# adamjorr/kbbq-py

Measured on NVIDIA B200. Metric: bases/sec recalibrated (table build + apply), higher is better.
Workload: dtype u8 in/out, u32->int64 counts, f64 model

## Files before the change

### include/kbbq_b200.h

```cpp
#ifndef KBBQ_B200_H
#define KBBQ_B200_H

#include <stddef.h>
#include <stdint.h>

#ifdef __cplusplus
extern "C" {
#endif

#define KBBQ_NQ 43
#define KBBQ_NDINUC 16

#define KBBQ_OK 0
#define KBBQ_E_ARG (-1)
#define KBBQ_E_CUDA (-2)
#define KBBQ_E_WORKSPACE (-3)
#define KBBQ_E_DATA (-4)
#define KBBQ_E_IO (-5)
#define KBBQ_E_FORMAT (-6)
#define KBBQ_E_RAGGED (-7)
#define KBBQ_E_NAME_FIELD (-8)
#define KBBQ_E_NAME_RG (-9)
#define KBBQ_E_NAME_MISMATCH (-10)
#define KBBQ_E_PEER (-11)
// ... 3 lines not shown
#define KBBQ_FLAG_BAD_BASE 2
#define KBBQ_FLAG_RG_RANGE 4
#define KBBQ_FLAG_SEGMENTS 8
#define KBBQ_FLAG_KMER_FULL 16

int kbbq_abi_version(void);
const char *kbbq_strerror(int code);
const char *kbbq_last_cuda_error(void);

int64_t kbbq_pos_table_elems(int L, int R);
int64_t kbbq_din_table_elems(int R);

int kbbq_workspace_bytes(int64_t N, int L, int R, size_t *bytes);

int kbbq_build(const uint8_t *seq_dev, const uint8_t *qual_dev, const uint8_t *corr_dev,
               const uint16_t *rg_dev, const uint8_t *second_dev, int64_t N, int L, int R,
               int minscore, int64_t *pos_errs_dev, int64_t *pos_total_dev, int64_t *din_errs_dev,
               int64_t *din_total_dev, void *workspace_dev, size_t workspace_bytes,
               int *status_dev, int path, void *stream);

int kbbq_marginals(const int64_t *pos_errs_dev, const int64_t *pos_total_dev, int L, int R,
                   int64_t *q_errs_dev, int64_t *q_total_dev, int64_t *rg_errs_dev,
                   int64_t *rg_total_dev, int64_t *meanq_dev, void *stream);

int kbbq_delta_q(const int64_t *prior_q_dev, const int64_t *numerrs_dev,
                 const int64_t *numtotal_dev, int64_t n, int64_t *delta_dev, void *stream);

int kbbq_posterior_q_real(const double *prior_q_dev, const int64_t *numerrs_dev,
                          const int64_t *numtotal_dev, int64_t n, int64_t *posterior_dev, void *stream);

int kbbq_bam_workspace_bytes(int64_t N, int L, int R, size_t *bytes);
int kbbq_build_bam(const uint8_t *seq_dev, const uint8_t *qual_dev, const uint8_t *err_dev,
                   const uint8_t *skip_dev, const uint16_t *rg_dev, const uint8_t *flags_dev,
                   const uint16_t *aln_start_dev, const uint16_t *aln_end_dev, int64_t N, int L, int R,
                   int minscore, int64_t *pos_errs_dev, int64_t *pos_total_dev, int64_t *din_errs_dev,
                   int64_t *din_total_dev, void *workspace_dev, size_t workspace_bytes, int *status_dev,
                   void *stream);
int kbbq_apply_bam(const uint8_t *seq_dev, const uint8_t *qual_dev, const uint16_t *rg_dev,
                   const uint8_t *flags_dev, int64_t N, int L, int R, int minscore,
                   const int64_t *meanq_dev, const int64_t *rgdq_dev, const int64_t *qdq_dev,
                   const int64_t *posdq_dev, const int64_t *dindq_dev, int nq, int ndin1,
                   uint8_t *out_qual_dev, void *workspace_dev, size_t workspace_bytes, int *status_dev,
                   void *stream);

int kbbq_calibration_counts(const uint8_t *qual_dev, const uint8_t *err_dev, const uint8_t *seq_dev,
                            const uint8_t *corr_dev, const uint8_t *skip_dev, int64_t n,
// ... 190 lines not shown
```

### kbbq-py_b200/csrc/host_api.cu

```cuda
#include <algorithm>
#include <atomic>
#include <chrono>
#include <condition_variable>
#include <memory>
#include <mutex>
#include <sched.h>
#include <stdlib.h>
#include <string.h>
#include <sys/mman.h>
#include <sys/stat.h>
#include <fcntl.h>
#include <thread>
#include <unistd.h>
#include <vector>

#include "common.cuh"

using namespace kbbq;

namespace {

#define KBBQ_TRY(x) do { int rc_ = (x); if (rc_) return rc_; } while (0)

constexpr int MAX_DEVICES = 16;
// ... 453 lines not shown
    if (st & KBBQ_FLAG_KMER_FULL) return KBBQ_E_DATA;
    S->kmer_t = min_count > 0 ? min_count : kbbq_kmer_min_count(hist);
    S->kmer_stage = KMER_READY;
    if (hist_out) memcpy(hist_out, hist, sizeof(hist));
    if (t_used) *t_used = S->kmer_t;
    return KBBQ_OK;
}

int build_chunk_kmer_async(kbbq_session *S, const uint8_t *seq, const uint8_t *qual, const uint16_t *rg,
                           const uint8_t *second, int64_t n) {
    if (S->kmer_stage != KMER_READY || n < 0 || n > S->C) return KBBQ_E_ARG;
    if (n == 0) return KBBQ_OK;
    if (!seq || !qual) return KBBQ_E_ARG;
    const int64_t k = S->built++;
    KBBQ_TRY(build_chunk_upload(S, k, seq, qual, rg, second, n, false, true));
    return build_chunk_finish(S, k, seq, nullptr, rg != nullptr, second != nullptr, n, false);
}

int model_async(kbbq_session *S) {
    const int L = S->L, R = S->R;
    const size_t npos = (size_t)R * NQ * 2 * L, ndin = (size_t)R * NQ * 16;
    int64_t *pe = S->summed ? S->d_sum : S->d_tab, *pt = pe + npos, *de = pt + npos, *dt = de + ndin;
    const ModelPtrs &mp = S->mp;
    KBBQ_TRY(kbbq_marginals(pe, pt, L, R, mp.q_errs, mp.q_total, mp.rg_errs, mp.rg_total, mp.meanq, S->s_comp));
    KBBQ_TRY(kbbq_get_delta_qs(mp.meanq, mp.rg_errs, mp.rg_total, mp.q_errs, mp.q_total, pe, pt, de, dt, R, NQ, 2 * L, 16,
                               mp.rgdq, mp.qdq, mp.posdq, mp.dindq, S->s_comp));
    return KBBQ_OK;
}

int apply_and_download(kbbq_session *S, const uint8_t *d_seq, const uint8_t *d_qual, const uint16_t *d_rg,
                       const uint8_t *d_sec, const uint32_t *seg, const uint32_t *dest, int64_t n, uint8_t *out_host) {
    const int L = S->L, R = S->R;
    OutSlot &o = S->down[S->applied++ & 1];
    const ModelPtrs &mp = S->mp;
    KBBQ_CUDA(cudaStreamWaitEvent(S->s_comp, o.drained, 0));
    if (S->segmode) {
        KBBQ_TRY(kbbq_apply_segmented(d_seq, d_qual, seg, S->rowsC, L, R, S->minscore, mp.meanq, mp.rgdq, mp.qdq, mp.posdq,
                                      mp.dindq, NQ, 17, o.out_seg, S->d_ws, S->ws_bytes, S->d_status, S->s_comp));
        KBBQ_TRY(kbbq_unsegment_rows(o.out_seg, dest, n, L, S->rowsC, o.out, S->s_comp));
    } else {
        KBBQ_TRY(kbbq_apply(d_seq, d_qual, d_rg, d_sec, n, L, R, S->minscore, mp.meanq, mp.rgdq, mp.qdq, mp.posdq, mp.dindq,
                            NQ, 17, o.out, S->d_ws, S->ws_bytes, S->d_status, 0, S->s_comp));
    }
    KBBQ_CUDA(cudaEventRecord(o.applied, S->s_comp));
    KBBQ_CUDA(cudaStreamWaitEvent(S->s_down, o.applied, 0));
    KBBQ_CUDA(cudaMemcpyAsync(out_host, o.out, (size_t)n * L, cudaMemcpyDeviceToHost, S->s_down));
    S->d2h_bytes += n * L;
    KBBQ_CUDA(cudaEventRecord(o.drained, S->s_down));
    return KBBQ_OK;
// ... 1058 lines not shown
    const auto d_hist = c.scratch(256 * sizeof(uint64_t));
    const auto d_tab = c.scratch(ntab * 8);
    const auto d_model = c.scratch(nmodel * 8);
    const auto ws = c.scratch(ws_bytes);
    const auto table = c.scratch(table_bytes);
    bool ok = false;
    KBBQ_TRY(c.fits(&ok));
    if (!ok) return KBBQ_E_UNSUPPORTED;
    KBBQ_TRY(c.begin());
    uint64_t hist[256];
    int t = 0, st = 0;
    const int rc = kmer_errors_dev(d_seq, N, L, k, min_count, table, cap, (uint64_t *)(void *)d_hist,
                                   (uint32_t *)(void *)d_bits, c.status, hist, &t, &st);
    if (rc == KBBQ_E_DATA && status_out) *status_out = st;
    KBBQ_TRY(rc);
    if (min_count_used) *min_count_used = t;
    int64_t *pe = (int64_t *)(void *)d_tab, *pt = pe + npos, *de = pt + npos, *dt = de + ndin;
    const ModelPtrs mp = carve_model((int64_t *)(void *)d_model, L, R);
    uint8_t *corr = (uint8_t *)(void *)d_corr;
    KBBQ_CUDA(cudaMemset(pe, 0, ntab * 8));
    KBBQ_TRY(kbbq_expand_mismatch_bits(d_seq, (uint32_t *)(void *)d_bits, (int64_t)nb, corr, nullptr));
    KBBQ_TRY(kbbq_build(d_seq, d_qual, corr, d_rg, d_sec, N, L, R, minscore, pe, pt, de, dt, ws, ws_bytes, c.status, 0,
                        nullptr));
    KBBQ_TRY(kbbq_marginals(pe, pt, L, R, mp.q_errs, mp.q_total, mp.rg_errs, mp.rg_total, mp.meanq, nullptr));
    KBBQ_TRY(kbbq_get_delta_qs(mp.meanq, mp.rg_errs, mp.rg_total, mp.q_errs, mp.q_total, pe, pt, de, dt, R, NQ, 2 * L,
                               16, mp.rgdq, mp.qdq, mp.posdq, mp.dindq, nullptr));
    KBBQ_TRY(kbbq_apply(d_seq, d_qual, d_rg, d_sec, N, L, R, minscore, mp.meanq, mp.rgdq, mp.qdq, mp.posdq, mp.dindq, NQ,
                        17, d_out, ws, ws_bytes, c.status, KBBQ_APPLY_BASES_CHECKED, nullptr));
    if (tables_host) KBBQ_CUDA(cudaMemcpy(tables_host, pe, ntab * 8, cudaMemcpyDeviceToHost));
    if (deltas_host)
        KBBQ_CUDA(cudaMemcpy(deltas_host, mp.meanq, ((size_t)2 * R + (size_t)R * NQ * (1 + 2 * L + 17)) * 8,
                             cudaMemcpyDeviceToHost));
    return c.finish(status_out);
}

}
```

### kbbq-py_b200/csrc/kbbq_b200.cu

```cuda
#include <algorithm>
#include <mutex>
#include <stdlib.h>
#include <string.h>
#include <vector>

#include "apply.cuh"
#include "bam.cuh"
#include "build.cuh"
#include "calib.cuh"
#include "common.cuh"
#include "expand.cuh"
#include "kmer.cuh"
#include "model.cuh"
#include "prepare.cuh"
#include "segment.cuh"
#include "synth.cuh"

namespace kbbq {

std::atomic<long long> g_launches{0};
char g_last_cuda_error[256] = "";

static std::mutex g_const_mu;
static bool g_const_done[64];
// ... 128 lines not shown
        return KBBQ_OK;
    }
    const int64_t tail = (R == 1 && N > p->g.G) ? N % p->g.G : 0;
    if (tail) {
        p->N = N - tail;
        rc = generic(p->N, tail, 1);
        if (rc) return rc;
    }
    return run_prepare(rg, second, p->N, p->g.G, R, p->w, status, p->sms, p->sl.ngs, p->g.gbytes, p->sl.slot, st);
}

template <class Launch>
static int launch_bam_chunks(long long N, int L, const Launch &launch) {
    const unsigned int wmax = (unsigned int)((3 + L + 3) >> 2);
    const long long per = std::max<long long>(1, (long long)(0x7FFFFFFFu / wmax) / 256 * 256);
    for (long long r0 = 0; r0 < N; r0 += per) {
        const long long n = std::min<long long>(per, N - r0);
        launch((unsigned)((n * wmax + BAM_WARPS * 32 - 1) / (BAM_WARPS * 32)), r0, wmax);
        KBBQ_LAUNCHED();
    }
    return KBBQ_OK;
}

}

using namespace kbbq;

extern "C" {

int kbbq_abi_version(void) { return 1; }

const char *kbbq_strerror(int code) {
    switch (code) {
    case KBBQ_OK: return "ok";
    case KBBQ_E_ARG: return "bad argument";
    case KBBQ_E_CUDA: return "CUDA runtime error";
    case KBBQ_E_WORKSPACE: return "workspace too small";
    case KBBQ_E_DATA: return "input data error (see status flags)";
    case KBBQ_E_IO: return "FASTQ file could not be opened, read or written";
    case KBBQ_E_FORMAT: return "malformed FASTQ (4-line records expected)";
    case KBBQ_E_RAGGED: return "reads of unequal length";
    case KBBQ_E_NAME_FIELD: return "read name has no read-group field";
    case KBBQ_E_NAME_RG: return "read-group field does not start with RG";
    case KBBQ_E_NAME_MISMATCH: return "corrected read name does not start with the read name";
    case KBBQ_E_PEER: return "multi-GPU: peer access between the devices is not available";
    case KBBQ_E_UNSUPPORTED: return "not handled by this entry point (use the chunked driver)";
// ... 64 lines not shown
}

int kbbq_build(const uint8_t *seq, const uint8_t *qual, const uint8_t *corr, const uint16_t *rg,
               const uint8_t *second, int64_t N, int L, int R, int minscore, int64_t *pos_errs,
               int64_t *pos_total, int64_t *din_errs, int64_t *din_total, void *workspace,
               size_t workspace_bytes, int *status, int path, void *stream) {
    return build_impl(seq, qual, corr, rg, second, N, L, R, minscore, pos_errs, pos_total, din_errs, din_total,
                      workspace, workspace_bytes, status, path, stream, nullptr);
}

int kbbq_build_segmented(const uint8_t *seq, const uint8_t *qual, const uint8_t *corr, const uint32_t *seg,
                         int64_t rows_bound, int L, int R, int minscore, int64_t *pos_errs, int64_t *pos_total,
                         int64_t *din_errs, int64_t *din_total, void *workspace, size_t workspace_bytes, int *status,
                         void *stream) {
    if (!seg || rows_bound % SEG_ALIGN) return KBBQ_E_ARG;
    return build_impl(seq, qual, corr, nullptr, nullptr, rows_bound, L, R, minscore, pos_errs, pos_total, din_errs,
                      din_total, workspace, workspace_bytes, status, 1, stream, seg);
}

int kbbq_marginals(const int64_t *pos_errs, const int64_t *pos_total, int L, int R, int64_t *q_errs,
                   int64_t *q_total, int64_t *rg_errs, int64_t *rg_total, int64_t *meanq, void *stream) {
    if (L < 1 || R < 1 || !pos_errs || !pos_total || !q_errs || !q_total || !rg_errs || !rg_total || !meanq)
        return KBBQ_E_ARG;
    cudaStream_t st = (cudaStream_t)stream;
    int rc = upload_constants();
    if (rc) return rc;
    marginals_q_kernel<<<dim3(NQ, R), 128, 0, st>>>((const long long *)pos_errs, (const long long *)pos_total,
                                                   2 * L, (long long *)q_errs, (long long *)q_total);
    KBBQ_LAUNCHED();
    marginals_rg_kernel<<<R, 64, 0, st>>>((const long long *)q_errs, (const long long *)q_total, R,
                                                      (long long *)rg_errs, (long long *)rg_total, (long long *)meanq);
    KBBQ_LAUNCHED();
    return KBBQ_OK;
}

int kbbq_delta_q(const int64_t *prior_q, const int64_t *numerrs, const int64_t *numtotal, int64_t n,
                 int64_t *delta, void *stream) {
    if (n < 0 || (n > 0 && (!prior_q || !numerrs || !numtotal || !delta))) return KBBQ_E_ARG;
    if (n == 0) return KBBQ_OK;
    int rc = upload_constants();
    if (rc) return rc;
    delta_q_kernel<<<(unsigned)((n + 127) / 128), 128, 0, (cudaStream_t)stream>>>(
        (const long long *)prior_q, (const long long *)numerrs, (const long long *)numtotal, n, (long long *)delta);
    KBBQ_LAUNCHED();
    return KBBQ_OK;
}

int kbbq_posterior_q_real(const double *prior_q, const int64_t *numerrs, const int64_t *numtotal, int64_t n,
                          int64_t *posterior, void *stream) {
    if (n < 0 || (n > 0 && (!prior_q || !numerrs || !numtotal || !posterior))) return KBBQ_E_ARG;
    if (n == 0) return KBBQ_OK;
    int rc = upload_constants();
    if (rc) return rc;
    posterior_q_real_kernel<<<(unsigned)((n + 127) / 128), 128, 0, (cudaStream_t)stream>>>(
        prior_q, (const long long *)numerrs, (const long long *)numtotal, n, (long long *)posterior);
    KBBQ_LAUNCHED();
// ... 126 lines not shown
    const long long chunk = (long long)grid * CAL_THREADS * CAL_MAX_ITERS * 32;
    auto kern = err ? (skip ? calibration_kernel<true, true> : calibration_kernel<true, false>)
                    : (skip ? calibration_kernel<false, true> : calibration_kernel<false, false>);
    KBBQ_CUDA(cudaFuncSetAttribute(kern, cudaFuncAttributeMaxDynamicSharedMemorySize, CAL_SMEM));
    for (long long o = 0; o < n; o += chunk) {
        CalibArgs c = a;
        c.qual += o; if (err) c.err += o; else { c.seq += o; c.corr += o; } if (skip) c.skip += o;
        c.n = std::min<long long>(chunk, n - o);
        kern<<<grid, CAL_THREADS, CAL_SMEM, st>>>(c);
        KBBQ_LAUNCHED();
    }
    return KBBQ_OK;
}

int kbbq_get_delta_qs(const int64_t *meanq, const int64_t *rg_errs, const int64_t *rg_total,
                      const int64_t *q_errs, const int64_t *q_total, const int64_t *pos_errs,
                      const int64_t *pos_total, const int64_t *din_errs, const int64_t *din_total, int R,
                      int nq, int ncyc, int ndin, int64_t *rgdq, int64_t *qdq, int64_t *posdq,
                      int64_t *dindq, void *stream) {
    if (R < 1 || nq < 1 || ncyc < 0 || ndin < 0) return KBBQ_E_ARG;
    if (!meanq || !rg_errs || !rg_total || !q_errs || !q_total || !rgdq || !qdq) return KBBQ_E_ARG;
    if ((ncyc && (!pos_errs || !pos_total || !posdq)) || !dindq || (ndin && (!din_errs || !din_total)))
        return KBBQ_E_ARG;
    int rc = upload_constants();
    if (rc) return rc;
    cudaStream_t st = (cudaStream_t)stream;
    DeltaArgs a = {(const long long *)meanq, (const long long *)rg_errs, (const long long *)rg_total,
                   (const long long *)q_errs, (const long long *)q_total, (const long long *)pos_errs,
                   (const long long *)pos_total, (const long long *)din_errs, (const long long *)din_total,
                   R, nq, ncyc, ndin, (long long *)rgdq, (long long *)qdq, (long long *)posdq, (long long *)dindq};
    delta_levels12_kernel<<<R, 64, 0, st>>>(a);
    KBBQ_LAUNCHED();
    const long long cells = (long long)R * nq * (ncyc + ndin + 1);
    delta_level3_kernel<<<(unsigned)((cells + 127) / 128), 128, 0, st>>>(a);
    KBBQ_LAUNCHED();
    return KBBQ_OK;
}

static int apply_impl(const uint8_t *seq, const uint8_t *qual, const uint16_t *rg, const uint8_t *second, int64_t N,
                      int L, int R, int minscore, const int64_t *meanq, const int64_t *rgdq, const int64_t *qdq,
                      const int64_t *posdq, const int64_t *dindq, int nq, int ndin1, uint8_t *out_qual,
                      void *workspace, size_t workspace_bytes, int *status, int path, void *stream,
                      const unsigned int *seg_rows) {
    const bool segmode = seg_rows != nullptr;
    const bool validate = !(path & KBBQ_APPLY_BASES_CHECKED);
    path &= ~KBBQ_APPLY_BASES_CHECKED;
    if (N < 0 || L < 1 || R < 1 || R > 65535 || minscore < 0 || minscore >= NQ) return KBBQ_E_ARG;
    if (nq < 1 || nq > NQ || ndin1 < 16 || ndin1 > 64) return KBBQ_E_ARG;
    if (!meanq || !rgdq || !qdq || !posdq || !dindq || !status) return KBBQ_E_ARG;
    if (N == 0) return KBBQ_OK;
    if (!seq || !qual || !out_qual) return KBBQ_E_ARG;
    cudaStream_t st = (cudaStream_t)stream;
    Workspace w = carve_workspace(workspace, N, L, R);
    if (!workspace || workspace_bytes < w.bytes) return KBBQ_E_WORKSPACE;

    const long long fold_cells = (long long)R * NQ * (2 * L + 16);
    fold_kernel<<<(unsigned)((fold_cells + 255) / 256), 256, 0, st>>>(
        (const long long *)meanq, (const long long *)rgdq, (const long long *)qdq, (const long long *)posdq,
        (const long long *)dindq, R, nq, 2 * L, ndin1, w.fold_cyc, w.fold_din);
// ... 321 lines not shown
```

### kbbq-py_b200/csrc/model.cuh

```cuda
#pragma once
#include "common.cuh"

namespace kbbq {

__constant__ double c_lnp[NQ];
__constant__ double c_ln1mp[NQ];
__constant__ double c_prior[NQ];
__constant__ double c_p[NQ];
__constant__ double c_bound_hi[NQ];
__constant__ double c_bound_lo[NQ];

struct dd { double hi, lo; };
__device__ __forceinline__ dd two_sum(double a, double b) {
    double s = __dadd_rn(a, b), bb = __dsub_rn(s, a);
    double e = __dadd_rn(__dsub_rn(a, __dsub_rn(s, bb)), __dsub_rn(b, bb));
    return {s, e};
}
__device__ __forceinline__ dd two_prod(double a, double b) {
    double p = __dmul_rn(a, b);
    return {p, __fma_rn(a, b, -p)};
}
__device__ __forceinline__ dd dd_add(dd a, dd b) {
    dd s = two_sum(a.hi, b.hi);
    double lo = __dadd_rn(s.lo, __dadd_rn(a.lo, b.lo));
    return two_sum(s.hi, lo);
}
__device__ __forceinline__ dd dd_div_d(dd a, double b) {
    double q1 = __ddiv_rn(a.hi, b);
    dd p = two_prod(q1, b);
    double r = __dadd_rn(__dsub_rn(__dsub_rn(a.hi, p.hi), p.lo), a.lo);
    double q2 = __ddiv_rn(r, b);
    return two_sum(q1, q2);
}
__device__ __forceinline__ bool dd_le(dd a, double bh, double bl) {
    return a.hi < bh || (a.hi == bh && a.lo <= bl);
}

__global__ void marginals_q_kernel(const long long *pos_errs, const long long *pos_total, int L2,
                                   long long *q_errs, long long *q_total) {
    const int q = blockIdx.x, rg = blockIdx.y;
    const size_t base = ((size_t)rg * NQ + q) * L2;
    long long e = 0, t = 0;
    for (int c = threadIdx.x; c < L2; c += blockDim.x) { e += pos_errs[base + c]; t += pos_total[base + c]; }
    __shared__ long long se[32], st[32];
    for (int o = 16; o; o >>= 1) { e += __shfl_down_sync(0xFFFFFFFFu, e, o); t += __shfl_down_sync(0xFFFFFFFFu, t, o); }
    if ((threadIdx.x & 31) == 0) { se[threadIdx.x >> 5] = e; st[threadIdx.x >> 5] = t; }
    __syncthreads();
    if (threadIdx.x == 0) {
        e = 0; t = 0;
        for (int w = 0; w < (blockDim.x + 31) / 32; ++w) { e += se[w]; t += st[w]; }
        q_errs[rg * NQ + q] = e;
        q_total[rg * NQ + q] = t;
    }
}

__global__ void marginals_rg_kernel(const long long *q_errs, const long long *q_total, int R,
                                    long long *rg_errs, long long *rg_total, long long *meanq) {
    const int rg = blockIdx.x;
    __shared__ long long s_e[NQ], s_t[NQ];
    if (threadIdx.x < NQ) {
        s_e[threadIdx.x] = q_errs[rg * NQ + threadIdx.x];
        s_t[threadIdx.x] = q_total[rg * NQ + threadIdx.x];
    }
    __syncthreads();
    if (threadIdx.x != 0) return;
    long long e = 0, t = 0;
    dd acc = {0.0, 0.0};
    for (int q = 0; q < NQ; ++q) {
        const long long tq = s_t[q];
        e += s_e[q];
        t += tq;
        if (tq) acc = dd_add(acc, two_prod((double)tq, c_p[q]));
    }
    rg_errs[rg] = e;
    rg_total[rg] = t;
    long long mq = 0;
    if (t > 0) {
        if (acc.hi == 0.0) mq = NQ - 1;
        else {
            const dd p = dd_div_d(acc, (double)t);
            for (int m = 1; m < NQ; ++m) mq += dd_le(p, c_bound_hi[m], c_bound_lo[m]) ? 1 : 0;
        }
    }
    meanq[rg] = mq;
}

__device__ __forceinline__ dd round_to_x87(dd s) {
    if (s.lo == 0.0 || isinf(s.hi) || isnan(s.hi)) return s;
    int e;
    frexp(s.hi, &e);
    int eh = e - 1;
    if (fabs(s.hi) == ldexp(1.0, eh) && ((s.hi > 0.0) != (s.lo > 0.0))) eh -= 1;
    const int qe = eh - 63;
    const double lo_r = ldexp(rint(ldexp(s.lo, -qe)), qe);
    const double h = __dadd_rn(s.hi, lo_r);
    return {h, __dadd_rn(__dsub_rn(s.hi, h), lo_r)};
}

template <typename PRIOR>
__device__ __forceinline__ int posterior_q_cell(PRIOR prior, long long errs, long long tot) {
    const double k = (double)(errs + 1), mm = (double)((tot + 2) - (errs + 1));
    int best = 0;
    double bh = 0.0, bl = 0.0;
    bool have = false;
    for (int c = 0; c < NQ; ++c) {
        int d = (int)((PRIOR)c - prior);
        d = d < 0 ? -d : d;
        const double pr = d < NQ ? c_prior[d] : -KBBQ_INF;
        const double a = __dmul_rn(k, c_lnp[c]);
        const double b = (mm == 0.0) ? 0.0 : __dmul_rn(mm, c_ln1mp[c]);
        const double ll = __dadd_rn(a, b);
        double h, l;
        if (isinf(pr) || isinf(ll)) { h = -KBBQ_INF; l = 0.0; }
        else { dd s = round_to_x87(two_sum(pr, ll)); h = s.hi; l = s.lo; }
        if (!have || h > bh || (h == bh && l > bl)) { best = c; bh = h; bl = l; have = true; }
    }
    return best;
}
__device__ __forceinline__ int delta_q_cell(int prior, long long errs, long long tot) {
    return posterior_q_cell<int>(prior, errs, tot) - prior;
}

__global__ void delta_q_kernel(const long long *prior, const long long *errs, const long long *tot,
                               long long n, long long *out) {
    long long i = (long long)blockIdx.x * blockDim.x + threadIdx.x;
    if (i < n) out[i] = delta_q_cell((int)prior[i], errs[i], tot[i]);
}

__global__ void posterior_q_real_kernel(const double *prior, const long long *errs, const long long *tot,
                                        long long n, long long *out) {
    long long i = (long long)blockIdx.x * blockDim.x + threadIdx.x;
    if (i < n) out[i] = posterior_q_cell<double>(prior[i], errs[i], tot[i]);
}

struct DeltaArgs {
    const long long *meanq, *rg_errs, *rg_total, *q_errs, *q_total, *pos_errs, *pos_total, *din_errs, *din_total;
    int R, nq, ncyc, ndin;
    long long *rgdq, *qdq, *posdq, *dindq;
};

__global__ void delta_levels12_kernel(DeltaArgs a) {
    const int rg = blockIdx.x;
    __shared__ int s_prior1;
    if (threadIdx.x == 0) {
        const int mq = (int)a.meanq[rg];
        const int d = delta_q_cell(mq, a.rg_errs[rg], a.rg_total[rg]);
        a.rgdq[rg] = d;
        s_prior1 = mq + d;
    }
    __syncthreads();
    for (int q = threadIdx.x; q < a.nq; q += blockDim.x)
        a.qdq[rg * a.nq + q] = delta_q_cell(s_prior1, a.q_errs[rg * a.nq + q], a.q_total[rg * a.nq + q]);
}

__global__ void delta_level3_kernel(DeltaArgs a) {
    const long long ncell_pos = (long long)a.R * a.nq * a.ncyc;
    const long long ncell_din = (long long)a.R * a.nq * (a.ndin + 1);
    long long i = (long long)blockIdx.x * blockDim.x + threadIdx.x;
    if (i < ncell_pos) {
        const long long gq = i / a.ncyc;
        const int rg = (int)(gq / a.nq);
        const int prior2 = (int)(a.meanq[rg] + a.rgdq[rg] + a.qdq[gq]);
        a.posdq[i] = delta_q_cell(prior2, a.pos_errs[i], a.pos_total[i]);
    } else if (i < ncell_pos + ncell_din) {
        i -= ncell_pos;
        const long long gq = i / (a.ndin + 1);
        const int d = (int)(i - gq * (a.ndin + 1));
        if (d == a.ndin) { a.dindq[i] = 0; return; }
        const int rg = (int)(gq / a.nq);
        const int prior2 = (int)(a.meanq[rg] + a.rgdq[rg] + a.qdq[gq]);
        a.dindq[i] = delta_q_cell(prior2, a.din_errs[gq * a.ndin + d], a.din_total[gq * a.ndin + d]);
    }
}

__global__ void fold_kernel(const long long *meanq, const long long *rgdq, const long long *qdq,
                            const long long *posdq, const long long *dindq, int R, int nq, int L2,
                            int ndin1, short *fold_cyc, short *fold_din) {
    const long long ncyc = (long long)R * NQ * L2, ndin = (long long)R * NQ * 16;
    long long i = (long long)blockIdx.x * blockDim.x + threadIdx.x;
    if (i < ncyc) {
        const long long gq = i / L2;
        const int c2 = (int)(i - gq * L2);
        const int rg = (int)(gq / NQ), q = (int)(gq - (long long)rg * NQ);
        long long v = 0;
        if (q < nq)
            v = meanq[rg] + rgdq[rg] + qdq[rg * nq + q] + posdq[((size_t)rg * nq + q) * L2 + c2] +
                dindq[((size_t)rg * nq + q) * ndin1 + ndin1 - 1];
        fold_cyc[i] = (short)v;
    } else if (i < ncyc + ndin) {
        i -= ncyc;
        const long long gq = i >> 4;
        const int n = (int)(i & 15);
        const int rg = (int)(gq / NQ), q = (int)(gq - (long long)rg * NQ);
        long long v = 0;
        if (q < nq) {
            const size_t row = ((size_t)rg * nq + q) * ndin1;
            v = dindq[row + nat_to_ref(n >> 2) * 4 + nat_to_ref(n & 3)] - dindq[row + ndin1 - 1];
// ... 7 lines not shown
```

### kbbq-py_b200/kbbq/_native.py

```python
import ctypes as C
import os

import numpy as np

HERE = os.path.dirname(os.path.abspath(__file__))
LIB_PATH = os.path.join(HERE, "libkbbq_b200.so")

NQ = 43
FLAG_QUAL_RANGE, FLAG_BAD_BASE, FLAG_RG_RANGE, FLAG_SEGMENTS = 1, 2, 4, 8
FLAG_KMER_FULL = 16
APPLY_BASES_CHECKED = 0x10
E_DATA = -4
E_UNSUPPORTED = -12

_lib = None

_vp, _i, _i64, _sz = C.c_void_p, C.c_int, C.c_int64, C.c_size_t
SIGNATURES = {
    "kbbq_abi_version": (_i, []),
    "kbbq_strerror": (C.c_char_p, [_i]),
    "kbbq_last_cuda_error": (C.c_char_p, []),
    "kbbq_pos_table_elems": (_i64, [_i, _i]),
    "kbbq_din_table_elems": (_i64, [_i]),
    "kbbq_workspace_bytes": (_i, [_i64, _i, _i, C.POINTER(_sz)]),
    "kbbq_build": (_i, [_vp] * 5 + [_i64, _i, _i, _i] + [_vp] * 4 + [_vp, _sz, _vp, _i, _vp]),
    "kbbq_marginals": (_i, [_vp, _vp, _i, _i] + [_vp] * 5 + [_vp]),
    "kbbq_delta_q": (_i, [_vp, _vp, _vp, _i64, _vp, _vp]),
    "kbbq_get_delta_qs": (_i, [_vp] * 9 + [_i, _i, _i, _i] + [_vp] * 4 + [_vp]),
    "kbbq_apply": (_i, [_vp] * 4 + [_i64, _i, _i, _i] + [_vp] * 5 + [_i, _i, _vp, _vp, _sz, _vp, _i, _vp]),
    "kbbq_recalibrate_host": (_i, [_vp] * 5 + [_i64, _i, _i, _i] + [_vp] * 3 + [C.POINTER(_i), _i]),
    "kbbq_recalibrate_host_multi": (_i, [_vp] * 5 + [_i64, _i, _i, _i] + [_vp] * 3 + [C.POINTER(_i), C.POINTER(_i), _i]),
    "kbbq_recalibrate_fastq": (_i, [C.c_char_p, C.c_char_p, _i, _i, _i, _i, _i, C.POINTER(_i64), C.POINTER(_i), C.POINTER(_i)]),
    "kbbq_host_release": (_i, [_i]),
    "kbbq_session_create": (_i, [_i, _i, _i, _i, _i64, _i64, _i, C.POINTER(_vp)]),
    "kbbq_session_destroy": (None, [_vp]),
    "kbbq_session_chunk_reads": (_i64, [_vp]),
    "kbbq_session_reset": (_i, [_vp]),
    "kbbq_session_build_chunk": (_i, [_vp] * 6 + [_i64, _i]),
    "kbbq_session_build_range": (_i, [_vp] * 6 + [_i64]),
    "kbbq_session_tables": (_i, [_vp, _vp]),
    "kbbq_session_set_tables": (_i, [_vp, _vp]),
    "kbbq_session_tables_dev": (_i, [_vp, C.POINTER(_vp), C.POINTER(_i64), C.POINTER(_vp)]),
    "kbbq_session_model": (_i, [_vp, _vp]),
    "kbbq_session_apply_resident": (_i, [_vp, _i64, _vp]),
    "kbbq_session_apply_chunk": (_i, [_vp] * 5 + [_i64, _vp]),
    "kbbq_session_flush": (_i, [_vp]),
    "kbbq_session_sync": (_i, [_vp, C.POINTER(_i)]),
    "kbbq_session_traffic": (_i, [_vp, C.POINTER(_i64), C.POINTER(_i64)]),
    "kbbq_build_host": (_i, [_vp] * 5 + [_i64, _i, _i, _i] + [_vp] * 4 + [C.POINTER(_i), _i]),
# ... 526 lines not shown
```

### kbbq-py_b200/kbbq/device.py

```python
import ctypes as C
import weakref

import torch

from . import _native
from . import parallel

NQ = _native.NQ


def _p(t):
    return None if t is None else C.c_void_p(t.data_ptr())


def _on_device(fn):
    import functools

    @functools.wraps(fn)
    def wrapper(self, *args, **kwargs):
        with torch.cuda.device(self.device):
            return fn(self, *args, **kwargs)
    return wrapper


# ... 116 lines not shown
        _native.check(rc)
        self._remember_built(sb.seq)

    @_on_device
    def apply_segmented(self, sb, out_seg):
        self._ensure_workspace(sb.rows_bound)
        flags = _native.APPLY_BASES_CHECKED if self._bases_checked(sb.seq) else 0
        rc = self.lib.kbbq_apply_segmented_flags(_p(sb.seq), _p(sb.qual), _p(sb.seg), sb.rows_bound, self.L, self.R,
                                                 self.minscore, _p(self.meanq), _p(self.rgdq), _p(self.qdq),
                                                 _p(self.posdq), _p(self.dindq), NQ, 17, _p(out_seg), _p(self.workspace),
                                                 self.ws_bytes, _p(self.status), flags, self._stream())
        _native.check(rc)

    @_on_device
    def unsegment(self, sb, out_seg, out):
        _native.check(self.lib.kbbq_unsegment_rows(_p(out_seg), _p(sb.dest), sb.N, self.L, sb.rows_bound, _p(out),
                                                   self._stream()))

    def allreduce(self):
        parallel.allreduce_tables(self.tables, self.pg)

    @_on_device
    def model(self):
        L, R = self.L, self.R
        _native.check(self.lib.kbbq_marginals(_p(self.pos_errs), _p(self.pos_total), L, R, _p(self.q_errs),
                                              _p(self.q_total), _p(self.rg_errs), _p(self.rg_total),
                                              _p(self.meanq), self._stream()))
        _native.check(self.lib.kbbq_get_delta_qs(_p(self.meanq), _p(self.rg_errs), _p(self.rg_total),
                                                 _p(self.q_errs), _p(self.q_total), _p(self.pos_errs),
                                                 _p(self.pos_total), _p(self.din_errs), _p(self.din_total),
                                                 R, NQ, 2 * L, 16, _p(self.rgdq), _p(self.qdq), _p(self.posdq),
                                                 _p(self.dindq), self._stream()))

    @_on_device
    def apply(self, seq, qual, out, rg=None, second=None, path=0):
        N = seq.numel() // self.L
        self._ensure_workspace(N)
        if self._bases_checked(seq):
            path |= _native.APPLY_BASES_CHECKED
        rc = self.lib.kbbq_apply(_p(seq), _p(qual), _p(rg), _p(second), N, self.L, self.R, self.minscore,
                                 _p(self.meanq), _p(self.rgdq), _p(self.qdq), _p(self.posdq), _p(self.dindq),
                                 NQ, 17, _p(out), _p(self.workspace), self.ws_bytes, _p(self.status), path,
                                 self._stream())
        _native.check(rc)

    @_on_device
    def build_bam(self, seq, qual, err, skip=None, rg=None, flags=None, aln_start=None, aln_end=None, fast=True):
        N = seq.numel() // self.L
        ws = self._bam_workspace(N) if fast else None
        rc = self.lib.kbbq_build_bam(_p(seq), _p(qual), _p(err), _p(skip), _p(rg), _p(flags), _p(aln_start),
                                     _p(aln_end), N, self.L, self.R, self.minscore, _p(self.pos_errs),
                                     _p(self.pos_total), _p(self.din_errs), _p(self.din_total), _p(ws),
                                     0 if ws is None else ws.numel(), _p(self.status), self._stream())
        _native.check(rc)

# ... 63 lines not shown
```

Baseline: 868.6 billion.

## Fuse marginals and delta-Q model into one multi-lane kernel

Replaces the four model-stage kernels (q marginals, rg marginals, levels 1-2 delta, level-3 delta) with one fused model_kernel. Each read-group block computes its marginals and prior chain in shared memory, and several blocks per read group split the level-3 cells. Each cell's posterior search over the quality candidates is spread across W warp lanes and reduced with shuffles, and the lookup tables are staged in shared memory. The aim is to cut launch overhead and the serial per-thread 43-candidate loop. In exchange, marginals and level 1-2 are recomputed redundantly in every block of a read group, and lane counts come from a heuristic.

```diff
diff --git a/include/kbbq_b200.h b/include/kbbq_b200.h
--- a/include/kbbq_b200.h
+++ b/include/kbbq_b200.h
@@ -49,6 +49,11 @@
 int kbbq_marginals(const int64_t *pos_errs_dev, const int64_t *pos_total_dev, int L, int R,
                    int64_t *q_errs_dev, int64_t *q_total_dev, int64_t *rg_errs_dev,
                    int64_t *rg_total_dev, int64_t *meanq_dev, void *stream);
+
+int kbbq_model(const int64_t *pos_errs_dev, const int64_t *pos_total_dev, const int64_t *din_errs_dev,
+               const int64_t *din_total_dev, int L, int R, int64_t *q_errs_dev, int64_t *q_total_dev,
+               int64_t *rg_errs_dev, int64_t *rg_total_dev, int64_t *meanq_dev, int64_t *rgdq_dev,
+               int64_t *qdq_dev, int64_t *posdq_dev, int64_t *dindq_dev, void *stream);
 
 int kbbq_delta_q(const int64_t *prior_q_dev, const int64_t *numerrs_dev,
                  const int64_t *numtotal_dev, int64_t n, int64_t *delta_dev, void *stream);
diff --git a/kbbq-py_b200/csrc/host_api.cu b/kbbq-py_b200/csrc/host_api.cu
--- a/kbbq-py_b200/csrc/host_api.cu
+++ b/kbbq-py_b200/csrc/host_api.cu
@@ -499,9 +499,8 @@
     const size_t npos = (size_t)R * NQ * 2 * L, ndin = (size_t)R * NQ * 16;
     int64_t *pe = S->summed ? S->d_sum : S->d_tab, *pt = pe + npos, *de = pt + npos, *dt = de + ndin;
     const ModelPtrs &mp = S->mp;
-    KBBQ_TRY(kbbq_marginals(pe, pt, L, R, mp.q_errs, mp.q_total, mp.rg_errs, mp.rg_total, mp.meanq, S->s_comp));
-    KBBQ_TRY(kbbq_get_delta_qs(mp.meanq, mp.rg_errs, mp.rg_total, mp.q_errs, mp.q_total, pe, pt, de, dt, R, NQ, 2 * L, 16,
-                               mp.rgdq, mp.qdq, mp.posdq, mp.dindq, S->s_comp));
+    KBBQ_TRY(kbbq_model(pe, pt, de, dt, L, R, mp.q_errs, mp.q_total, mp.rg_errs, mp.rg_total, mp.meanq, mp.rgdq, mp.qdq,
+                        mp.posdq, mp.dindq, S->s_comp));
     return KBBQ_OK;
 }
 
@@ -1606,9 +1605,8 @@
     KBBQ_TRY(kbbq_expand_mismatch_bits(d_seq, (uint32_t *)(void *)d_bits, (int64_t)nb, corr, nullptr));
     KBBQ_TRY(kbbq_build(d_seq, d_qual, corr, d_rg, d_sec, N, L, R, minscore, pe, pt, de, dt, ws, ws_bytes, c.status, 0,
                         nullptr));
-    KBBQ_TRY(kbbq_marginals(pe, pt, L, R, mp.q_errs, mp.q_total, mp.rg_errs, mp.rg_total, mp.meanq, nullptr));
-    KBBQ_TRY(kbbq_get_delta_qs(mp.meanq, mp.rg_errs, mp.rg_total, mp.q_errs, mp.q_total, pe, pt, de, dt, R, NQ, 2 * L,
-                               16, mp.rgdq, mp.qdq, mp.posdq, mp.dindq, nullptr));
+    KBBQ_TRY(kbbq_model(pe, pt, de, dt, L, R, mp.q_errs, mp.q_total, mp.rg_errs, mp.rg_total, mp.meanq, mp.rgdq, mp.qdq,
+                        mp.posdq, mp.dindq, nullptr));
     KBBQ_TRY(kbbq_apply(d_seq, d_qual, d_rg, d_sec, N, L, R, minscore, mp.meanq, mp.rgdq, mp.qdq, mp.posdq, mp.dindq, NQ,
                         17, d_out, ws, ws_bytes, c.status, KBBQ_APPLY_BASES_CHECKED, nullptr));
     if (tables_host) KBBQ_CUDA(cudaMemcpy(tables_host, pe, ntab * 8, cudaMemcpyDeviceToHost));
diff --git a/kbbq-py_b200/csrc/kbbq_b200.cu b/kbbq-py_b200/csrc/kbbq_b200.cu
--- a/kbbq-py_b200/csrc/kbbq_b200.cu
+++ b/kbbq-py_b200/csrc/kbbq_b200.cu
@@ -174,6 +174,32 @@
     return KBBQ_OK;
 }
 
+template <bool MARG>
+static int launch_model(ModelArgs a, cudaStream_t st) {
+    int rc = upload_constants();
+    if (rc) return rc;
+    int device, sms, max_smem;
+    rc = current_device_info(&device, &sms, &max_smem);
+    if (rc) return rc;
+    const long long cells = a.rgdq ? (long long)a.nq * (a.ncyc + a.ndin + 1) : 0;
+    const long long slots = (long long)sms * MODEL_THREADS;
+    int W = 1;
+    while (cells && W < 32 && (long long)a.R * cells * (2 * W) <= slots) W *= 2;
+    if (const char *e = getenv("KBBQ_MODEL_LANES")) {
+        const int f = atoi(e);
+        if (f >= 1 && f <= 32 && !(f & (f - 1))) W = f;
+    }
+    a.lanes = W;
+    a.cpr = (int)std::min(std::max(1LL, (cells * W + MODEL_THREADS - 1) / MODEL_THREADS), std::max(1LL, 2LL * sms / a.R));
+    const size_t smem = sizeof(int) * (size_t)a.nq;
+    if (smem + 4096 > (size_t)max_smem) return KBBQ_E_ARG;
+    if (smem > 49152)
+        KBBQ_CUDA(cudaFuncSetAttribute(model_kernel<MARG>, cudaFuncAttributeMaxDynamicSharedMemorySize, (int)smem));
+    model_kernel<MARG><<<(unsigned)a.R * a.cpr, MODEL_THREADS, smem, st>>>(a);
+    KBBQ_LAUNCHED();
+    return KBBQ_OK;
+}
+
 }
 
 using namespace kbbq;
@@ -284,16 +310,23 @@
                    int64_t *q_total, int64_t *rg_errs, int64_t *rg_total, int64_t *meanq, void *stream) {
     if (L < 1 || R < 1 || !pos_errs || !pos_total || !q_errs || !q_total || !rg_errs || !rg_total || !meanq)
         return KBBQ_E_ARG;
-    cudaStream_t st = (cudaStream_t)stream;
-    int rc = upload_constants();
-    if (rc) return rc;
-    marginals_q_kernel<<<dim3(NQ, R), 128, 0, st>>>((const long long *)pos_errs, (const long long *)pos_total,
-                                                   2 * L, (long long *)q_errs, (long long *)q_total);
-    KBBQ_LAUNCHED();
-    marginals_rg_kernel<<<R, 64, 0, st>>>((const long long *)q_errs, (const long long *)q_total, R,
-                                                      (long long *)rg_errs, (long long *)rg_total, (long long *)meanq);
-    KBBQ_LAUNCHED();
-    return KBBQ_OK;
+    ModelArgs a = {(const long long *)pos_errs, (const long long *)pos_total, nullptr, nullptr, (long long *)q_errs,
+                   (long long *)q_total, (long long *)rg_errs, (long long *)rg_total, (long long *)meanq,
+                   nullptr, nullptr, nullptr, nullptr, R, NQ, 2 * L, 16, 1, 1};
+    return launch_model<true>(a, (cudaStream_t)stream);
+}
+
+int kbbq_model(const int64_t *pos_errs, const int64_t *pos_total, const int64_t *din_errs, const int64_t *din_total,
+               int L, int R, int64_t *q_errs, int64_t *q_total, int64_t *rg_errs, int64_t *rg_total, int64_t *meanq,
+               int64_t *rgdq, int64_t *qdq, int64_t *posdq, int64_t *dindq, void *stream) {
+    if (L < 1 || R < 1 || !pos_errs || !pos_total || !din_errs || !din_total || !q_errs || !q_total || !rg_errs ||
+        !rg_total || !meanq || !rgdq || !qdq || !posdq || !dindq)
+        return KBBQ_E_ARG;
+    ModelArgs a = {(const long long *)pos_errs, (const long long *)pos_total, (const long long *)din_errs,
+                   (const long long *)din_total, (long long *)q_errs, (long long *)q_total, (long long *)rg_errs,
+                   (long long *)rg_total, (long long *)meanq, (long long *)rgdq, (long long *)qdq, (long long *)posdq,
+                   (long long *)dindq, R, NQ, 2 * L, 16, 1, 1};
+    return launch_model<true>(a, (cudaStream_t)stream);
 }
 
 int kbbq_delta_q(const int64_t *prior_q, const int64_t *numerrs, const int64_t *numtotal, int64_t n,
@@ -466,19 +499,11 @@
     if (!meanq || !rg_errs || !rg_total || !q_errs || !q_total || !rgdq || !qdq) return KBBQ_E_ARG;
     if ((ncyc && (!pos_errs || !pos_total || !posdq)) || !dindq || (ndin && (!din_errs || !din_total)))
         return KBBQ_E_ARG;
-    int rc = upload_constants();
-    if (rc) return rc;
-    cudaStream_t st = (cudaStream_t)stream;
-    DeltaArgs a = {(const long long *)meanq, (const long long *)rg_errs, (const long long *)rg_total,
-                   (const long long *)q_errs, (const long long *)q_total, (const long long *)pos_errs,
-                   (const long long *)pos_total, (const long long *)din_errs, (const long long *)din_total,
-                   R, nq, ncyc, ndin, (long long *)rgdq, (long long *)qdq, (long long *)posdq, (long long *)dindq};
-    delta_levels12_kernel<<<R, 64, 0, st>>>(a);
-    KBBQ_LAUNCHED();
-    const long long cells = (long long)R * nq * (ncyc + ndin + 1);
-    delta_level3_kernel<<<(unsigned)((cells + 127) / 128), 128, 0, st>>>(a);
-    KBBQ_LAUNCHED();
-    return KBBQ_OK;
+    ModelArgs a = {(const long long *)pos_errs, (const long long *)pos_total, (const long long *)din_errs,
+                   (const long long *)din_total, (long long *)q_errs, (long long *)q_total, (long long *)rg_errs,
+                   (long long *)rg_total, (long long *)meanq, (long long *)rgdq, (long long *)qdq, (long long *)posdq,
+                   (long long *)dindq, R, nq, ncyc, ndin, 1, 1};
+    return launch_model<false>(a, (cudaStream_t)stream);
 }
 
 static int apply_impl(const uint8_t *seq, const uint8_t *qual, const uint16_t *rg, const uint8_t *second, int64_t N,
diff --git a/kbbq-py_b200/csrc/model.cuh b/kbbq-py_b200/csrc/model.cuh
--- a/kbbq-py_b200/csrc/model.cuh
+++ b/kbbq-py_b200/csrc/model.cuh
@@ -34,55 +34,6 @@
 }
 __device__ __forceinline__ bool dd_le(dd a, double bh, double bl) {
     return a.hi < bh || (a.hi == bh && a.lo <= bl);
-}
-
-__global__ void marginals_q_kernel(const long long *pos_errs, const long long *pos_total, int L2,
-                                   long long *q_errs, long long *q_total) {
-    const int q = blockIdx.x, rg = blockIdx.y;
-    const size_t base = ((size_t)rg * NQ + q) * L2;
-    long long e = 0, t = 0;
-    for (int c = threadIdx.x; c < L2; c += blockDim.x) { e += pos_errs[base + c]; t += pos_total[base + c]; }
-    __shared__ long long se[32], st[32];
-    for (int o = 16; o; o >>= 1) { e += __shfl_down_sync(0xFFFFFFFFu, e, o); t += __shfl_down_sync(0xFFFFFFFFu, t, o); }
-    if ((threadIdx.x & 31) == 0) { se[threadIdx.x >> 5] = e; st[threadIdx.x >> 5] = t; }
-    __syncthreads();
-    if (threadIdx.x == 0) {
-        e = 0; t = 0;
-        for (int w = 0; w < (blockDim.x + 31) / 32; ++w) { e += se[w]; t += st[w]; }
-        q_errs[rg * NQ + q] = e;
-        q_total[rg * NQ + q] = t;
-    }
-}
-
-__global__ void marginals_rg_kernel(const long long *q_errs, const long long *q_total, int R,
-                                    long long *rg_errs, long long *rg_total, long long *meanq) {
-    const int rg = blockIdx.x;
-    __shared__ long long s_e[NQ], s_t[NQ];
-    if (threadIdx.x < NQ) {
-        s_e[threadIdx.x] = q_errs[rg * NQ + threadIdx.x];
-        s_t[threadIdx.x] = q_total[rg * NQ + threadIdx.x];
-    }
-    __syncthreads();
-    if (threadIdx.x != 0) return;
-    long long e = 0, t = 0;
-    dd acc = {0.0, 0.0};
-    for (int q = 0; q < NQ; ++q) {
-        const long long tq = s_t[q];
-        e += s_e[q];
-        t += tq;
-        if (tq) acc = dd_add(acc, two_prod((double)tq, c_p[q]));
-    }
-    rg_errs[rg] = e;
-    rg_total[rg] = t;
-    long long mq = 0;
-    if (t > 0) {
-        if (acc.hi == 0.0) mq = NQ - 1;
-        else {
-            const dd p = dd_div_d(acc, (double)t);
-            for (int m = 1; m < NQ; ++m) mq += dd_le(p, c_bound_hi[m], c_bound_lo[m]) ? 1 : 0;
-        }
-    }
-    meanq[rg] = mq;
 }
 
 __device__ __forceinline__ dd round_to_x87(dd s) {
@@ -97,28 +48,53 @@
     return {h, __dadd_rn(__dsub_rn(s.hi, h), lo_r)};
 }
 
+
+struct ModelTabs { const double *lnp, *ln1mp, *prior; };
+
+template <typename PRIOR>
+__device__ __forceinline__ dd posterior_candidate(const ModelTabs &t, int c, PRIOR prior, double k, double mm) {
+    int d = (int)((PRIOR)c - prior);
+    d = d < 0 ? -d : d;
+    const double pr = d < NQ ? t.prior[d] : -KBBQ_INF;
+    const double a = __dmul_rn(k, t.lnp[c]);
+    const double b = (mm == 0.0) ? 0.0 : __dmul_rn(mm, t.ln1mp[c]);
+    const double ll = __dadd_rn(a, b);
+    if (isinf(pr) || isinf(ll)) return {-KBBQ_INF, 0.0};
+    return round_to_x87(two_sum(pr, ll));
+}
+
 template <typename PRIOR>
 __device__ __forceinline__ int posterior_q_cell(PRIOR prior, long long errs, long long tot) {
+    const ModelTabs t = {c_lnp, c_ln1mp, c_prior};
     const double k = (double)(errs + 1), mm = (double)((tot + 2) - (errs + 1));
     int best = 0;
     double bh = 0.0, bl = 0.0;
     bool have = false;
     for (int c = 0; c < NQ; ++c) {
-        int d = (int)((PRIOR)c - prior);
-        d = d < 0 ? -d : d;
-        const double pr = d < NQ ? c_prior[d] : -KBBQ_INF;
-        const double a = __dmul_rn(k, c_lnp[c]);
-        const double b = (mm == 0.0) ? 0.0 : __dmul_rn(mm, c_ln1mp[c]);
-        const double ll = __dadd_rn(a, b);
-        double h, l;
-        if (isinf(pr) || isinf(ll)) { h = -KBBQ_INF; l = 0.0; }
-        else { dd s = round_to_x87(two_sum(pr, ll)); h = s.hi; l = s.lo; }
-        if (!have || h > bh || (h == bh && l > bl)) { best = c; bh = h; bl = l; have = true; }
+        const dd s = posterior_candidate(t, c, prior, k, mm);
+        if (!have || s.hi > bh || (s.hi == bh && s.lo > bl)) { best = c; bh = s.hi; bl = s.lo; have = true; }
     }
     return best;
 }
 __device__ __forceinline__ int delta_q_cell(int prior, long long errs, long long tot) {
     return posterior_q_cell<int>(prior, errs, tot) - prior;
+}
+
+__device__ __forceinline__ int posterior_q_lanes(const ModelTabs &t, int prior, long long errs, long long tot, int W,
+                                                 int j) {
+    const double k = (double)(errs + 1), mm = (double)((tot + 2) - (errs + 1));
+    int best = j;
+    dd b = posterior_candidate(t, j, prior, k, mm);
+    for (int c = j + W; c < NQ; c += W) {
+        const dd s = posterior_candidate(t, c, prior, k, mm);
+        if (s.hi > b.hi || (s.hi == b.hi && s.lo > b.lo)) { best = c; b = s; }
+    }
+    for (int o = W >> 1; o; o >>= 1) {
+        const double oh = __shfl_xor_sync(0xFFFFFFFFu, b.hi, o), ol = __shfl_xor_sync(0xFFFFFFFFu, b.lo, o);
+        const int oc = __shfl_xor_sync(0xFFFFFFFFu, best, o);
+        if (oh > b.hi || (oh == b.hi && (ol > b.lo || (ol == b.lo && oc < best)))) { b.hi = oh; b.lo = ol; best = oc; }
+    }
+    return best;
 }
 
 __global__ void delta_q_kernel(const long long *prior, const long long *errs, const long long *tot,
@@ -133,46 +109,136 @@
     if (i < n) out[i] = posterior_q_cell<double>(prior[i], errs[i], tot[i]);
 }
 
-struct DeltaArgs {
-    const long long *meanq, *rg_errs, *rg_total, *q_errs, *q_total, *pos_errs, *pos_total, *din_errs, *din_total;
+struct ModelArgs {
+    const long long *pos_errs, *pos_total, *din_errs, *din_total;
+    long long *q_errs, *q_total, *rg_errs, *rg_total, *meanq;
+    long long *rgdq, *qdq, *posdq, *dindq;
     int R, nq, ncyc, ndin;
-    long long *rgdq, *qdq, *posdq, *dindq;
+    int cpr;
+    int lanes;
 };
 
-__global__ void delta_levels12_kernel(DeltaArgs a) {
-    const int rg = blockIdx.x;
+constexpr int MODEL_THREADS = 512;
+constexpr int MODEL_L2_LANES = 8;
+
+template <bool MARG>
+__global__ void __launch_bounds__(MODEL_THREADS, 2) model_kernel(ModelArgs a) {
+    __shared__ double s_tab[3][NQ];
+    __shared__ long long s_qe[NQ], s_qt[NQ];
     __shared__ int s_prior1;
-    if (threadIdx.x == 0) {
-        const int mq = (int)a.meanq[rg];
-        const int d = delta_q_cell(mq, a.rg_errs[rg], a.rg_total[rg]);
-        a.rgdq[rg] = d;
-        s_prior1 = mq + d;
+    extern __shared__ int s_prior2[];
+    const int rg = blockIdx.x / a.cpr, part = blockIdx.x - rg * a.cpr;
+    const bool lead = part == 0;
+    const int tid = threadIdx.x, lane = tid & 31, warp = tid >> 5, nwarps = blockDim.x >> 5;
+    for (int i = tid; i < NQ; i += blockDim.x) {
+        s_tab[0][i] = c_lnp[i];
+        s_tab[1][i] = c_ln1mp[i];
+        s_tab[2][i] = c_prior[i];
+    }
+    const ModelTabs t = {s_tab[0], s_tab[1], s_tab[2]};
+    if (MARG) {
+        for (int q = warp; q < NQ; q += nwarps) {
+            const size_t base = ((size_t)rg * NQ + q) * a.ncyc;
+            long long e = 0, n = 0;
+            for (int c = lane; c < a.ncyc; c += 32) { e += a.pos_errs[base + c]; n += a.pos_total[base + c]; }
+            for (int o = 16; o; o >>= 1) { e += __shfl_xor_sync(0xFFFFFFFFu, e, o); n += __shfl_xor_sync(0xFFFFFFFFu, n, o); }
+            if (lane == 0) { s_qe[q] = e; s_qt[q] = n; }
+        }
     }
     __syncthreads();
-    for (int q = threadIdx.x; q < a.nq; q += blockDim.x)
-        a.qdq[rg * a.nq + q] = delta_q_cell(s_prior1, a.q_errs[rg * a.nq + q], a.q_total[rg * a.nq + q]);
-}
-
-__global__ void delta_level3_kernel(DeltaArgs a) {
-    const long long ncell_pos = (long long)a.R * a.nq * a.ncyc;
-    const long long ncell_din = (long long)a.R * a.nq * (a.ndin + 1);
-    long long i = (long long)blockIdx.x * blockDim.x + threadIdx.x;
-    if (i < ncell_pos) {
-        const long long gq = i / a.ncyc;
-        const int rg = (int)(gq / a.nq);
-        const int prior2 = (int)(a.meanq[rg] + a.rgdq[rg] + a.qdq[gq]);
-        a.posdq[i] = delta_q_cell(prior2, a.pos_errs[i], a.pos_total[i]);
-    } else if (i < ncell_pos + ncell_din) {
-        i -= ncell_pos;
-        const long long gq = i / (a.ndin + 1);
-        const int d = (int)(i - gq * (a.ndin + 1));
-        if (d == a.ndin) { a.dindq[i] = 0; return; }
-        const int rg = (int)(gq / a.nq);
-        const int prior2 = (int)(a.meanq[rg] + a.rgdq[rg] + a.qdq[gq]);
-        a.dindq[i] = delta_q_cell(prior2, a.din_errs[gq * a.ndin + d], a.din_total[gq * a.ndin + d]);
-    }
-}
-
+    if (MARG && lead)
+        for (int q = tid; q < NQ; q += blockDim.x) { a.q_errs[rg * NQ + q] = s_qe[q]; a.q_total[rg * NQ + q] = s_qt[q]; }
+
+    if (warp == 0) {
+        long long mq = 0, e = 0, n = 0;
+        if (MARG) {
+            if (lane == 0) {
+                dd acc = {0.0, 0.0};
+                for (int q = 0; q < NQ; ++q) {
+                    const long long tq = s_qt[q];
+                    e += s_qe[q];
+                    n += tq;
+                    if (tq) acc = dd_add(acc, two_prod((double)tq, c_p[q]));
+                }
+                if (n > 0) {
+                    if (acc.hi == 0.0) mq = NQ - 1;
+                    else {
+                        const dd p = dd_div_d(acc, (double)n);
+                        for (int m = 1; m < NQ; ++m) mq += dd_le(p, c_bound_hi[m], c_bound_lo[m]) ? 1 : 0;
+                    }
+                }
+                if (lead) { a.rg_errs[rg] = e; a.rg_total[rg] = n; a.meanq[rg] = mq; }
+            }
+            mq = __shfl_sync(0xFFFFFFFFu, mq, 0);
+            e = __shfl_sync(0xFFFFFFFFu, e, 0);
+            n = __shfl_sync(0xFFFFFFFFu, n, 0);
+        } else {
+            mq = a.meanq[rg];
+            e = a.rg_errs[rg];
+            n = a.rg_total[rg];
+        }
+        if (a.rgdq) {
+            const int p0 = (int)mq;
+            const int d = posterior_q_lanes(t, p0, e, n, 32, lane) - p0;
+            if (lane == 0) {
+                s_prior1 = p0 + d;
+                if (lead) a.rgdq[rg] = d;
+            }
+        }
+    }
+    if (!a.rgdq) return;
+    __syncthreads();
+
+    const int p1 = s_prior1;
+    {
+        constexpr int W2 = MODEL_L2_LANES, per = 32 / W2;
+        const int j = lane & (W2 - 1);
+        for (int q0 = warp * per; q0 < a.nq; q0 += nwarps * per) {
+            const int q = q0 + lane / W2;
+            long long e = 0, n = 0;
+            if (q < a.nq) {
+                if (MARG) { e = s_qe[q]; n = s_qt[q]; }
+                else { e = a.q_errs[rg * a.nq + q]; n = a.q_total[rg * a.nq + q]; }
+            }
+            const int d = posterior_q_lanes(t, p1, e, n, W2, j) - p1;
+            if (q < a.nq && j == 0) {
+                s_prior2[q] = p1 + d;
+                if (lead) a.qdq[rg * a.nq + q] = d;
+            }
+        }
+    }
+    __syncthreads();
+
+    const long long npos = (long long)a.nq * a.ncyc, ncell = npos + (long long)a.nq * (a.ndin + 1);
+    const long long chunk = (ncell + a.cpr - 1) / a.cpr;
+    const long long lo = part * chunk, hi = lo + chunk < ncell ? lo + chunk : ncell;
+    const int W = a.lanes, per = 32 / W, j = lane & (W - 1);
+    for (long long c0 = lo + (long long)warp * per; c0 < hi; c0 += (long long)nwarps * per) {
+        const long long i = c0 + lane / W;
+        long long e = 0, n = 0, *out = nullptr;
+        int prior = 0;
+        bool pad = false;
+        if (i < hi) {
+            if (i < npos) {
+                const size_t g = (size_t)rg * npos + i;
+                e = a.pos_errs[g];
+                n = a.pos_total[g];
+                prior = s_prior2[i / a.ncyc];
+                out = a.posdq + g;
+            } else {
+                const long long k = i - npos;
+                const int q = (int)(k / (a.ndin + 1)), d = (int)(k - (long long)q * (a.ndin + 1));
+                const size_t row = (size_t)rg * a.nq + q;
+                prior = s_prior2[q];
+                out = a.dindq + row * (a.ndin + 1) + d;
+                pad = d == a.ndin;
+                if (!pad) { e = a.din_errs[row * a.ndin + d]; n = a.din_total[row * a.ndin + d]; }
+            }
+        }
+        const int c = posterior_q_lanes(t, prior, e, n, W, j);
+        if (out && j == 0) *out = pad ? 0 : c - prior;
+    }
+}
 __global__ void fold_kernel(const long long *meanq, const long long *rgdq, const long long *qdq,
                             const long long *posdq, const long long *dindq, int R, int nq, int L2,
                             int ndin1, short *fold_cyc, short *fold_din) {
diff --git a/kbbq-py_b200/kbbq/_native.py b/kbbq-py_b200/kbbq/_native.py
--- a/kbbq-py_b200/kbbq/_native.py
+++ b/kbbq-py_b200/kbbq/_native.py
@@ -25,6 +25,7 @@
     "kbbq_workspace_bytes": (_i, [_i64, _i, _i, C.POINTER(_sz)]),
     "kbbq_build": (_i, [_vp] * 5 + [_i64, _i, _i, _i] + [_vp] * 4 + [_vp, _sz, _vp, _i, _vp]),
     "kbbq_marginals": (_i, [_vp, _vp, _i, _i] + [_vp] * 5 + [_vp]),
+    "kbbq_model": (_i, [_vp] * 4 + [_i, _i] + [_vp] * 9 + [_vp]),
     "kbbq_delta_q": (_i, [_vp, _vp, _vp, _i64, _vp, _vp]),
     "kbbq_get_delta_qs": (_i, [_vp] * 9 + [_i, _i, _i, _i] + [_vp] * 4 + [_vp]),
     "kbbq_apply": (_i, [_vp] * 4 + [_i64, _i, _i, _i] + [_vp] * 5 + [_i, _i, _vp, _vp, _sz, _vp, _i, _vp]),
diff --git a/kbbq-py_b200/kbbq/device.py b/kbbq-py_b200/kbbq/device.py
--- a/kbbq-py_b200/kbbq/device.py
+++ b/kbbq-py_b200/kbbq/device.py
@@ -162,15 +162,10 @@
 
     @_on_device
     def model(self):
-        L, R = self.L, self.R
-        _native.check(self.lib.kbbq_marginals(_p(self.pos_errs), _p(self.pos_total), L, R, _p(self.q_errs),
-                                              _p(self.q_total), _p(self.rg_errs), _p(self.rg_total),
-                                              _p(self.meanq), self._stream()))
-        _native.check(self.lib.kbbq_get_delta_qs(_p(self.meanq), _p(self.rg_errs), _p(self.rg_total),
-                                                 _p(self.q_errs), _p(self.q_total), _p(self.pos_errs),
-                                                 _p(self.pos_total), _p(self.din_errs), _p(self.din_total),
-                                                 R, NQ, 2 * L, 16, _p(self.rgdq), _p(self.qdq), _p(self.posdq),
-                                                 _p(self.dindq), self._stream()))
+        _native.check(self.lib.kbbq_model(_p(self.pos_errs), _p(self.pos_total), _p(self.din_errs), _p(self.din_total),
+                                          self.L, self.R, _p(self.q_errs), _p(self.q_total), _p(self.rg_errs),
+                                          _p(self.rg_total), _p(self.meanq), _p(self.rgdq), _p(self.qdq),
+                                          _p(self.posdq), _p(self.dindq), self._stream()))
 
     @_on_device
     def apply(self, seq, qual, out, rg=None, second=None, path=0):
```

After: 894.9 billion (median of 6 runs). 1.03x the previous value.
